# kcheng1021/UC-NeRF

Hardware: AMD Instinct MI355X
Metric: rays/sec (fwd render), 1280x1920 @ 64+128 samples (higher is better)
Workload: dtype f32-class (dense layers: f16 MFMA on hi/lo-split f32 operands, 2^-22 per product, f32 accumulate; grid, resampling, compositing f32)

## Files before the change

ucnerf_amd/_lib.py:

```python
import ctypes
import os

import torch

_HERE = os.path.dirname(os.path.abspath(__file__))
LIB_PATH = os.environ.get("UCN_LIB_PATH") or os.path.join(_HERE, "csrc", "libucnerf_march.so")
ABI_VERSION = 26
LAUNCH_CORESIDENT = 0x100
TABLE_F16 = 0x200
RAYS_INCOHERENT = 0x1000
GFEAT_LEVEL_MAJOR4 = 0x20000
GFEAT_LEVEL_MAJOR = 0x10000
BWD_FIXED_POINT = 0x800
FEATURES_BF16 = 0x400
FEAT_BF16 = 0x100

c_u32, c_u64, c_i32, c_f32, c_vp = ctypes.c_uint32, ctypes.c_uint64, ctypes.c_int, ctypes.c_float, ctypes.c_void_p


class UcnField(ctypes.Structure):
    _fields_ = [
        ("embeddings", c_vp), ("offsets_host", c_vp), ("grid_sizes_host", c_vp),
        ("num_levels", c_u32), ("level_dim", c_u32), ("base_resolution", c_u32),
        ("log2_per_level_scale", c_f32),
        ("w_d0", c_vp), ("b_d0", c_vp), ("w_d1", c_vp), ("b_d1", c_vp),
        ("n_bottleneck", c_u32),
        ("w_c0", c_vp), ("b_c0", c_vp), ("w_c1", c_vp), ("b_c1", c_vp), ("w_rgb", c_vp), ("b_rgb", c_vp),
        ("n_width", c_u32), ("n_dir", c_u32),
        ("density_bias", c_f32), ("rgb_premultiplier", c_f32), ("rgb_bias", c_f32), ("rgb_padding", c_f32),
        ("packed", c_vp),
        ("mlp_mode", c_u32),
    ]


class UcnSky(ctypes.Structure):
    _fields_ = [
        ("w_pts", c_vp * 8), ("b_pts", c_vp * 8),
        ("w_alpha", c_vp), ("b_alpha", c_vp), ("w_feat", c_vp), ("b_feat", c_vp),
        ("w_view", c_vp), ("b_view", c_vp), ("w_rgb", c_vp), ("b_rgb", c_vp),
        ("packed", c_vp),
# ... 155 lines not shown
```

ucnerf_amd/csrc/field_mlp.hip:

```cpp
#include "field_plan.h"
#include "wave_dpp.h"

namespace {

__global__ __launch_bounds__(256) void k_pack_first(const float *__restrict__ W, uint32_t F, float *__restrict__ dst) {
    const uint32_t i = blockIdx.x * 256u + threadIdx.x;
    const uint32_t KQ = F / 2;
    if (i >= 2u * KQ * 64u) return;
    const uint32_t lane = i & 63u, q = (i >> 6) % KQ, ot = (i >> 6) / KQ;
    dst[i] = W[(size_t)(32u * ot + (lane & 31u)) * F + 2u * q + (lane >> 5)];
}

constexpr int kMaxDir = 27;
template <int NW>
__global__ __launch_bounds__(256) void k_dir_bias(const float *__restrict__ viewdirs, const float *__restrict__ wc0,
                                                  const float *__restrict__ wc1, uint32_t nb, uint32_t ndir,
                                                  uint32_t N, float *__restrict__ out) {
    constexpr int RB = 16;
    constexpr int GROUPS = 256 / NW;
    __shared__ float enc[RB][kMaxDir + 1];
    const uint32_t ray0 = blockIdx.x * RB;
    const uint32_t deg = (ndir - 3u) / 6u;
    for (uint32_t i = threadIdx.x; i < RB * ndir; i += 256u) {
        const uint32_t rl = i / ndir, k = i - rl * ndir;
// ... 96 lines not shown
    init_bias<NTB>(x, a.b_d1, nullptr, h);
    chain<NTB, 2>(G1, x, h0, ws);
    if (live && h == 0) a.density[out_index(a, b)] = softplus(x[0][0] + a.density_bias);
    if (a.bott && live) {
#pragma unroll
        for (int t = 0; t < NTB; t++)
#pragma unroll
            for (int r = 0; r < 16; r++) a.bott[(size_t)out_index(a, b) * (NTB * 32) + acc_row(t, r, h)] = x[t][r];
    }
    if (a.rgb == nullptr) {
        ws.drain();
        __syncthreads();
        return;
    }
    const float *db = a.dir_bias + (size_t)ray_index(a, b) * 2 * (NTW * 32);
    f32x16 h2[NTW];
    init_bias<NTW>(h2, a.b_c1, db + NTW * 32, h);
    chain<NTW, NTB>(G2, h2, x, ws);
    hidden_tiles<0, NTB, NTW>(G3, PER_TILE, h2, x, a.b_c0, db, h, ws);
    rgb_head<NTW>(h2, a, b, live, h);
}

}

extern "C" uint64_t ucn_field_packed_floats(const ucn_field_t *f) {
    PackPlan pl;
    if (make_plan(f, &pl)) return 0;
    return pl.total;
}

extern "C" uint64_t ucn_field_dir_floats(const ucn_field_t *f, uint32_t N) {
    PackPlan pl;
    if (make_plan(f, &pl) || pl.prop) return 0;
    return f->mlp_mode == 1 ? (uint64_t)N * 32 : (uint64_t)N * 2 * f->n_width;
}

extern "C" int ucn_field_pack(const ucn_field_t *f, ucn_stream_t stream) {
    PackPlan pl;
    if (int rc = make_plan(f, &pl)) return rc;
    UCN_REQUIRE(f->packed && f->w_d0 && f->w_d1 && f->b_d0 && f->b_d1, "field_pack: density MLP weights / packed buffer missing");
    hipStream_t st = (hipStream_t)stream;
    if (!pl.prop && f->mlp_mode == 1) return ucn_h_pack(f, pl, st);
    hipLaunchKernelGGL(k_pack_first, dim3(ucn_div_up(2ull * pl.KQ * 64, 256)), dim3(256), 0, st, f->w_d0, pl.F, f->packed + pl.p0);
    if (pl.prop) {
        hipLaunchKernelGGL(k_pack_head, dim3(1), dim3(256), 0, st, f->w_d1, 64u, 0u, 64u, 1u, 1u, f->packed + pl.phead);
    } else {
        const uint32_t NB = f->n_bottleneck, NW = f->n_width, ND = f->n_dir;
        uint64_t off = pl.pstream;
        auto chainpack = [&](const float *W, uint32_t ld, uint32_t col0, uint32_t row_tile0, uint32_t nto, uint32_t nti) {
            hipLaunchKernelGGL(k_pack_chain, dim3(ucn_div_up((uint64_t)nto * nti * 1024, 256)), dim3(256), 0, st, W, ld,
                               col0, row_tile0, nto, nti, f->packed + off);
            off += (uint64_t)nto * nti * 1024;
        };
        chainpack(f->w_d1, 64, 0, 0, pl.NTB, 2);
        chainpack(f->w_c1, NW + NB + ND, NW, 0, pl.NTW, pl.NTB);
        for (uint32_t t = 0; t < pl.NTW; t++) {
            chainpack(f->w_c0, NB + ND, 0, t, 1, pl.NTB);
            chainpack(f->w_c1, NW + NB + ND, 32 * t, 0, pl.NTW, 1);
        }
        const uint64_t end = pl.pstream + (uint64_t)pl.n_groups * 256;
        if (off < end)
            hipLaunchKernelGGL(k_fill_zero, dim3(ucn_div_up(end - off, 256)), dim3(256), 0, st, f->packed + off, (uint32_t)(end - off));
        hipLaunchKernelGGL(k_pack_head, dim3(ucn_div_up((uint64_t)NW * 4, 256)), dim3(256), 0, st, f->w_rgb, NW, 0u, NW,
                           3u, 4u, f->packed + pl.phead);
    }
    UCN_LAUNCH_CHECK("field_pack");
    return 0;
}

extern "C" int ucn_field_dir_bias(const ucn_field_t *f, const float *viewdirs, uint32_t N, float *dir_bias_out,
                                  ucn_stream_t stream) {
    PackPlan pl;
    if (int rc = make_plan(f, &pl)) return rc;
    UCN_REQUIRE(!pl.prop, "field_dir_bias: field has no colour MLP (disable_rgb)");
    UCN_REQUIRE(N == 0 || (viewdirs && dir_bias_out), "field_dir_bias: null pointer argument");
    UCN_REQUIRE((f->n_dir - 3) % 6 == 0, "field_dir_bias: n_dir must be 3+6*deg, got %u", f->n_dir);
    if (N == 0) return 0;
    hipStream_t st = (hipStream_t)stream;
    if (f->mlp_mode == 1) return ucn_h_dir_enc(f, viewdirs, N, dir_bias_out, st);
    const dim3 grid(ucn_div_up(N, 16));
    if (f->n_width == 256)
        hipLaunchKernelGGL(k_dir_bias<256>, grid, dim3(256), 0, st, viewdirs, f->w_c0, f->w_c1, f->n_bottleneck, f->n_dir, N, dir_bias_out);
    else
        hipLaunchKernelGGL(k_dir_bias<64>, grid, dim3(256), 0, st, viewdirs, f->w_c0, f->w_c1, f->n_bottleneck, f->n_dir, N, dir_bias_out);
    UCN_LAUNCH_CHECK("field_dir_bias");
    return 0;
}

static thread_local const uint32_t *g_mlp_idx = nullptr, *g_mlp_count = nullptr;

extern "C" int ucn_field_mlp(const ucn_field_t *f, const float *features, uint32_t B, uint32_t samples_per_ray,
                             int rays_fastest, const float *dir_bias, float *density_out, float *rgb_out,
                             float *bottleneck_out, ucn_stream_t stream) {
    PackPlan pl;
    if (int rc = make_plan(f, &pl)) return rc;
    UCN_REQUIRE(B == 0 || (features && density_out && f->packed), "field_mlp: null pointer argument");
    UCN_REQUIRE(samples_per_ray >= 1, "field_mlp: samples_per_ray must be >= 1");
    UCN_REQUIRE(pl.prop ? rgb_out == nullptr : true, "field_mlp: a disable_rgb field has no colour output");
    UCN_REQUIRE(B == 0 || rgb_out == nullptr || dir_bias != nullptr, "field_mlp: colour output needs the per-ray direction terms");
    if (B == 0) return 0;
    MlpArgs a;
    a.feat = features; a.packed = f->packed;
    a.b_d0 = f->b_d0; a.b_d1 = f->b_d1; a.b_c0 = f->b_c0; a.b_c1 = f->b_c1; a.b_rgb = f->b_rgb;
    a.dir_bias = dir_bias; a.density = density_out; a.rgb = rgb_out; a.bott = bottleneck_out;
    UCN_REQUIRE(!(rays_fastest & 1) || B % samples_per_ray == 0, "field_mlp: B must be rays x samples_per_ray");
    a.B = B; a.spr = samples_per_ray; a.C = f->level_dim; a.F = pl.F;
    a.cshift = 0xFFu;
    if ((a.C == 1 || a.C == 2 || a.C == 4 || a.C == 8) && (uint64_t)B * a.C * (pl.F / a.C + 2) < (1ull << 30))
        a.cshift = a.C == 1 ? 0u : a.C == 2 ? 1u : a.C == 4 ? 2u : 3u;
    a.n_rays = B / samples_per_ray; a.rays_fastest = (rays_fastest & 1) ? 1u : 0u;
    a.small_ring = (rays_fastest & UCN_LAUNCH_CORESIDENT) ? 1u : 0u;
    a.idx = g_mlp_idx; a.count = g_mlp_count;
    a.n_chunks = pl.n_groups / kChunkGroups;
    a.p0 = pl.p0; a.pstream = pl.pstream; a.phead = pl.phead;
    a.density_bias = f->density_bias; a.rgb_premult = f->rgb_premultiplier; a.rgb_bias = f->rgb_bias;
    a.rgb_padding = f->rgb_padding;
    const dim3 grid(ucn_div_up(B, 128));
    hipStream_t st = (hipStream_t)stream;
    const size_t lds = 2 * kChunkGroups * 256 * sizeof(float);
    if (pl.prop) hipLaunchKernelGGL(k_prop_mlp, grid, dim3(256), 0, st, a);
    else if (f->mlp_mode == 1) return ucn_h_launch(pl, a, grid, st);
    else if (pl.NTB == 8) hipLaunchKernelGGL((k_field_mlp<8, 8>), grid, dim3(256), lds, st, a);
    else hipLaunchKernelGGL((k_field_mlp<2, 2>), grid, dim3(256), lds, st, a);
    UCN_LAUNCH_CHECK("field_mlp");
    return 0;
}

extern "C" int ucn_field_rgb_compacted(const ucn_field_t *f, const float *features, uint32_t B, uint32_t samples_per_ray,
                                       int rays_fastest, const float *dir_bias, const uint32_t *idx, const uint32_t *count,
                                       float *rgb_out, ucn_stream_t stream) {
    UCN_REQUIRE(f && f->mlp_mode == 1 && f->n_bottleneck != 1, "field_rgb_compacted: needs a colour field in mlp_mode 1");
    UCN_REQUIRE(B == 0 || (idx && count && rgb_out), "field_rgb_compacted: null pointer argument");
    g_mlp_idx = idx; g_mlp_count = count;
    const int rc = ucn_field_mlp(f, features, B, samples_per_ray, rays_fastest, dir_bias, rgb_out, rgb_out, nullptr, stream);
    g_mlp_idx = g_mlp_count = nullptr;
    return rc;
}
```

ucnerf_amd/csrc/field_mlp_h.hip:

```cpp
#include "field_plan.h"
#include "wave_dpp.h"
#include "mlp_ring.h"

namespace {

constexpr int kKS = (int)kFirstSteps;
constexpr int kDirExp = 10;
enum { E_IN = 0, E_H0 = 1, E_H1 = 2, E_H2 = 3, E_COUNT = 4 };

__global__ __launch_bounds__(256) void k_dir_enc(const float *__restrict__ viewdirs, uint32_t ndir, uint32_t N,
                                                 float *__restrict__ out) {
    const uint32_t i = blockIdx.x * 256u + threadIdx.x;
    if (i >= N * 32u) return;
    const uint32_t ray = i >> 5, k = i & 31u;
    const uint32_t deg = (ndir - 3u) / 6u;
    float v;
    if (k < 3u) {
        v = viewdirs[ray * 3 + k];
    } else if (k < ndir) {
        const uint32_t kk = (k - 3u) % (3u * deg), a = kk % 3u, si = kk / 3u;
        const float sc = viewdirs[ray * 3 + a] * (float)(1u << si);
        v = (k - 3u) < 3u * deg ? sinf(sc) : sinf(sc + 1.5707963705062866f);
    } else {
        v = k == ndir ? 1.0f : 0.0f;
    }
    out[i] = ldexpf(v, kDirExp);
}

__global__ __launch_bounds__(256) void k_compose(const float *__restrict__ Wout, uint32_t ldo, uint32_t col0,
                                                 const float *__restrict__ bias_out, const float *__restrict__ Wd1,
                                                 const float *__restrict__ bd1, uint32_t NB, uint32_t ND, uint32_t NW,
                                                 float *__restrict__ M) {
    const uint32_t i = blockIdx.x * 256u + threadIdx.x;
    if (i >= NW * kCompCols) return;
    const uint32_t j = i / kCompCols, c = i - j * kCompCols;
    const float *wr = Wout + (size_t)j * ldo + col0;
    float v = 0.0f;
    if (c < 64u) {
        double acc = 0.0;
        for (uint32_t k = 0; k < NB; k++) acc += (double)wr[k] * (double)Wd1[(size_t)k * 64 + c];
        v = (float)acc;
    } else if (c - 64u < ND) {
        v = wr[NB + c - 64u];
    } else if (c == 64u + ND) {
        double acc = (double)bias_out[j];
        for (uint32_t k = 0; k < NB; k++) acc += (double)wr[k] * (double)bd1[k];
        v = (float)acc;
    }
    M[i] = v;
}

__global__ __launch_bounds__(256) void k_absmax(const float *__restrict__ x, uint64_t n, uint32_t *__restrict__ out_bits) {
    float m = 0.0f;
    for (uint64_t i = (uint64_t)blockIdx.x * 256u + threadIdx.x; i < n; i += (uint64_t)gridDim.x * 256u) {
        const float v = fabsf(x[i]);
        m = v > m ? v : m;
    }
#pragma unroll
    for (int o = 32; o > 0; o >>= 1) m = fmaxf(m, __shfl_xor(m, o, 64));
// ... 158 lines not shown
#else
#define UCN_STAMP(i) do { } while (0)
#endif
template <int NTW, bool RGB, int CHUNK, int STAGE>
__global__ __launch_bounds__(256) void k_field_mlp_h(MlpArgs a) {
#ifdef UCN_EXP_TIMING
    const unsigned long long t_begin = __builtin_readcyclecounter();
#endif
    extern __shared__ __attribute__((aligned(16))) float s_lds[];
    const int lane = threadIdx.x & 63;
    const int wave = __builtin_amdgcn_readfirstlane(threadIdx.x >> 6);
    const int j = lane & 31, h = lane >> 5;
    const uint32_t b0 = (blockIdx.x * 4u + wave) * 32u;
    bool live = b0 + j < a.B;
    uint32_t b = live ? b0 + j : a.B - 1;
    if (a.idx) {
        const uint32_t cnt = *a.count;
        if (blockIdx.x * 128u >= cnt) return;
        live = b0 + j < cnt;
        b = a.idx[live ? b0 + j : cnt - 1];
    }
    const uint32_t oi = out_index(a, b);

    constexpr int NP = NTW / 2;
    constexpr int GA = 4 * kKS;
    constexpr int GB = GA + NP * 24;
    constexpr int PB = 24 + NTW * 8;
    constexpr int NG = RGB ? GB + NP * PB : GA;

    float fv[kKS][8];
    load_features<kKS>(a, b, h, fv);
    f32x16 ev;
    if constexpr (RGB) {
        const float4 *ep = reinterpret_cast<const float4 *>(a.dir_bias + (size_t)ray_index(a, b) * 32 + 4 * h);
#pragma unroll
        for (int r4 = 0; r4 < 4; r4++) {
            const float4 v = ep[2 * r4];
            ev[4 * r4 + 0] = v.x; ev[4 * r4 + 1] = v.y; ev[4 * r4 + 2] = v.z; ev[4 * r4 + 3] = v.w;
        }
    }
    const float *side = s_lds;
    Ring<NG, CHUNK, 4, kRingSlots, kLead, STAGE> ring(a.packed + a.pstream + kSideGroups * 256, s_lds + kSideGroups * 256, lane, wave);
    {
        const uint32_t lbase = (uint32_t)(size_t)(__attribute__((address_space(3))) float *)s_lds;
#pragma unroll
        for (int i = 0; i < kSideGroups / 4; i++)
            dma_group(a.packed + a.pstream + (size_t)(i * 4 + wave) * 256, lbase + (uint32_t)(i * 4 + wave) * 1024u, (uint32_t)lane * 16u);
    }
    rstatic_for<kLead>([&](auto c) { ring.template issue_chunk<c.value>(); });
    UCN_STAMP(0);
    if constexpr (STAGE > 0) ring.drain();
    ring.template boundary<0>();
    UCN_STAMP(1);
    if constexpr (RGB) {
#pragma unroll
        for (int r = 0; r < 16; r++) asm volatile("" : "+v"(ev[r]));
    }
    const float in_scale = side[129];

    f32x16 acc0[2];
#pragma unroll
    for (int t = 0; t < 2; t++) {
        const float4 *pb = reinterpret_cast<const float4 *>(side + t * 32 + h * 16);
#pragma unroll
        for (int r4 = 0; r4 < 4; r4++) {
            const float4 v = pb[r4];
            acc0[t][4 * r4 + 0] = v.x; acc0[t][4 * r4 + 1] = v.y; acc0[t][4 * r4 + 2] = v.z; acc0[t][4 * r4 + 3] = v.w;
// ... 68 lines not shown
                    dstep<G, NG>(acc[qp][0], acc[qp][1], in[i / 2].hi[i % 2], in[i / 2].lo[i % 2], pipe, ring);
            });
            UCN_STAMP(5 + 2 * p);
            rstatic_for<2 * NTW>([&](auto ic) {
                constexpr int i = ic.value, G = GB + p * PB + 24 + i * 4;
                if constexpr (p > 0 && i < 2)
                    dstep<G, NG, 3, 4>(acc[qp][0], acc[qp][1], h1s[i / 2].hi[i % 2], h1s[i / 2].lo[i % 2], pipe, ring,
                                       [&] { head_eighth<2 * (p - 1), 6 + i>(acc[qq], side, h, s0, s1, s2); });
                else
                    dstep<G, NG>(acc[qp][0], acc[qp][1], h1s[i / 2].hi[i % 2], h1s[i / 2].lo[i % 2], pipe, ring);
            });
            UCN_STOP_AT(3 + p, acc[qp]);
        });
        UCN_STAMP(13);
        rstatic_for<8>([&](auto e) { head_eighth<2 * (NP - 1), e.value>(acc[(2 * NP - 1) % 2], side, h, s0, s1, s2); });
        UCN_STAMP(14);
        s0 = xor32_sum(s0);
        s1 = xor32_sum(s1);
        s2 = xor32_sum(s2);
        if (live && h == 0) {
            const float pad = a.rgb_padding;
            const float v[3] = {s0 + a.b_rgb[0], s1 + a.b_rgb[1], s2 + a.b_rgb[2]};
            const size_t o = (size_t)oi * 3;
#pragma unroll
            for (int c = 0; c < 3; c++) {
                const float sg = 1.0f / (1.0f + expf(-(a.rgb_premult * v[c] + a.rgb_bias)));
                a.rgb[o + c] = sg * (1.0f + 2.0f * pad) - pad;
            }
        }
    }
}


template <int NTW, int NWAVES, int CHUNK, int SLOTS, int LEAD, int DEPTH>
__global__ __launch_bounds__(NWAVES * 64, 2) void k_field_mlp_h8(MlpArgs a) {
#ifdef UCN_EXP_TIMING
    const unsigned long long t_begin = __builtin_readcyclecounter();
#define UCN_STAMP8(i) do { if (blockIdx.x == UCN_EXP_TIMING && (threadIdx.x & 255) == 0) a.bott[(threadIdx.x >> 8) * 32 + (i)] = (float)(__builtin_readcyclecounter() - t_begin); } while (0)
#else
#define UCN_STAMP8(i) do { } while (0)
#endif
    extern __shared__ __attribute__((aligned(16))) float s_lds[];
    const int lane = threadIdx.x & 63;
    const int wave = __builtin_amdgcn_readfirstlane(threadIdx.x >> 6);
    const int j = lane & 31, h = lane >> 5;
    const uint32_t b0 = (blockIdx.x * NWAVES + wave) * 32u;
    bool live = b0 + j < a.B;
    uint32_t b = live ? b0 + j : a.B - 1;
    if (a.idx) {
        const uint32_t cnt = *a.count;
        if (blockIdx.x * (NWAVES * 32u) >= cnt) return;
        live = b0 + j < cnt;
        b = a.idx[live ? b0 + j : cnt - 1];
    }
    const uint32_t oi = out_index(a, b);
    constexpr int NP = NTW / 2;
    constexpr int GA = 4 * kKS;
    constexpr int GB = GA + NP * 24;
    constexpr int PB = 24 + NTW * 8;
    constexpr int NG = GB + NP * PB;

    float fv[kKS][8];
    load_features<kKS>(a, b, h, fv);
    f32x16 ev;
    {
        const float4 *ep = reinterpret_cast<const float4 *>(a.dir_bias + (size_t)ray_index(a, b) * 32 + 4 * h);
#pragma unroll
        for (int r4 = 0; r4 < 4; r4++) {
            const float4 v = ep[2 * r4];
            ev[4 * r4 + 0] = v.x; ev[4 * r4 + 1] = v.y; ev[4 * r4 + 2] = v.z; ev[4 * r4 + 3] = v.w;
        }
    }
    const float *side = s_lds;
    Ring<NG, CHUNK, NWAVES, SLOTS, LEAD> ring(a.packed + a.pstream + kSideGroups * 256, s_lds + kSideGroups * 256, lane, wave);
    {
        const uint32_t lbase = (uint32_t)(size_t)(__attribute__((address_space(3))) float *)s_lds;
#pragma unroll
        for (int i = 0; i < kSideGroups / NWAVES; i++)
            dma_group(a.packed + a.pstream + (size_t)(i * NWAVES + wave) * 256, lbase + (uint32_t)(i * NWAVES + wave) * 1024u, (uint32_t)lane * 16u);
    }
    UCN_STAMP8(0);
    rstatic_for<LEAD>([&](auto c) { ring.template issue_chunk<c.value>(); });
    UCN_STAMP8(1);
    ring.template boundary<0>();
    UCN_STAMP8(2);
#pragma unroll
    for (int r = 0; r < 16; r++) asm volatile("" : "+v"(ev[r]));
    const float in_scale = side[129];

    f32x16 acc[2];
#pragma unroll
    for (int t = 0; t < 2; t++) {
        const float4 *pb = reinterpret_cast<const float4 *>(side + t * 32 + h * 16);
#pragma unroll
        for (int r4 = 0; r4 < 4; r4++) {
            const float4 v = pb[r4];
            acc[t][4 * r4 + 0] = v.x; acc[t][4 * r4 + 1] = v.y; acc[t][4 * r4 + 2] = v.z; acc[t][4 * r4 + 3] = v.w;
        }
    }
    OpPipeD<DEPTH> pipe;
    pipe_prime_d<NG>(pipe, ring);
    {
        h8 fhi[kKS], flo[kKS];
#pragma unroll
        for (int s = 0; s < kKS; s++) {
#pragma unroll
            for (int e = 0; e < 8; e++) fv[s][e] *= in_scale;
            rsplit8(fv[s], fhi[s], flo[s]);
        }
        rstatic_for<kKS>([&](auto s) { dstep_d<4 * s.value, NG>(acc[0], acc[1], fhi[s.value], flo[s.value], pipe, ring); });
    }
    {
        const float *pd = side + 64;
        float part = 0.0f;
#pragma unroll
        for (int it = 0; it < 2; it++)
#pragma unroll
            for (int r = 0; r < 16; r++) part = fmaf(relu_bits(acc[it][r]), pd[(it * 16 + r) * 2 + h], part);
        const float raw = xor32_sum(part) + pd[64];
        if (live && h == 0 && a.idx == nullptr) a.density[oi] = softplus(raw + a.density_bias);
    }
    UCN_STAMP8(3);
    HPair in[3];
#pragma unroll
    for (int s = 0; s < 2; s++) {
        split_half<true>(acc[0], s, in[0]);
        split_half<true>(acc[1], s, in[1]);
        split_half<false>(ev, s, in[2]);
    }
    UCN_STAMP8(4);
    HPair h1s[NTW];
    rstatic_for<NP>([&](auto pc) {
        constexpr int p = pc.value;
#pragma unroll
        for (int r = 0; r < 16; r++) acc[0][r] = acc[1][r] = 0.0f;
        rstatic_for<6>([&](auto ic) {
            constexpr int i = ic.value, G = GA + (p * 6 + i) * 4;
            dstep_d<G, NG>(acc[0], acc[1], in[i / 2].hi[i % 2], in[i / 2].lo[i % 2], pipe, ring);
        });
#pragma unroll
        for (int s = 0; s < 2; s++) {
            split_half<true>(acc[0], s, h1s[2 * p]);
            split_half<true>(acc[1], s, h1s[2 * p + 1]);
        }
    });
    UCN_STAMP8(5);
    float s0 = 0.0f, s1 = 0.0f, s2 = 0.0f;
    rstatic_for<NP>([&](auto pc) {
        constexpr int p = pc.value;
#pragma unroll
        for (int r = 0; r < 16; r++) acc[0][r] = acc[1][r] = 0.0f;
        rstatic_for<6>([&](auto ic) {
            constexpr int i = ic.value, G = GB + p * PB + i * 4;
            dstep_d<G, NG>(acc[0], acc[1], in[i / 2].hi[i % 2], in[i / 2].lo[i % 2], pipe, ring);
        });
        rstatic_for<2 * NTW>([&](auto ic) {
            constexpr int i = ic.value, G = GB + p * PB + 24 + i * 4;
            dstep_d<G, NG>(acc[0], acc[1], h1s[i / 2].hi[i % 2], h1s[i / 2].lo[i % 2], pipe, ring);
        });
        UCN_STAMP8(6 + 2 * p);
        rstatic_for<8>([&](auto e) { head_eighth<2 * p, e.value>(acc, side, h, s0, s1, s2); });
        UCN_STAMP8(7 + 2 * p);
    });
    s0 = xor32_sum(s0);
    s1 = xor32_sum(s1);
    s2 = xor32_sum(s2);
    if (live && h == 0) {
        const float pad = a.rgb_padding;
        const float v[3] = {s0 + a.b_rgb[0], s1 + a.b_rgb[1], s2 + a.b_rgb[2]};
        const size_t o = (size_t)oi * 3;
#pragma unroll
        for (int c = 0; c < 3; c++) {
            const float sg = 1.0f / (1.0f + expf(-(a.rgb_premult * v[c] + a.rgb_bias)));
            a.rgb[o + c] = sg * (1.0f + 2.0f * pad) - pad;
        }
    }
}

}

int ucn_h_pack(const ucn_field_t *f, const PackPlan &pl, hipStream_t st) {
    const uint32_t NB = f->n_bottleneck, NW = f->n_width, ND = f->n_dir;
    float *side = f->packed + pl.pstream;
    float *stream = side + kSideGroups * 256;
    float *MA = f->packed + pl.pcomp, *MB = MA + (size_t)NW * kCompCols;
    float *scratch = MB + (size_t)NW * kCompCols;
    int *exps = reinterpret_cast<int *>(scratch + 1);
    const uint64_t n_floats = (uint64_t)pl.n_groups * 256;
    hipLaunchKernelGGL(k_fill_zero, dim3(ucn_div_up(n_floats, 256)), dim3(256), 0, st, side, (uint32_t)n_floats);
    hipLaunchKernelGGL(k_fill_zero, dim3(1), dim3(256), 0, st, scratch, 16u);
    const dim3 cg(ucn_div_up((uint64_t)NW * kCompCols, 256));
    hipLaunchKernelGGL(k_compose, cg, dim3(256), 0, st, f->w_c0, NB + ND, 0u, f->b_c0, f->w_d1, f->b_d1, NB, ND, NW, MA);
    hipLaunchKernelGGL(k_compose, cg, dim3(256), 0, st, f->w_c1, NW + NB + ND, NW, f->b_c1, f->w_d1, f->b_d1, NB, ND, NW, MB);
    const uint64_t n_emb = (uint64_t)f->offsets_host[f->num_levels] * f->level_dim;
    hipLaunchKernelGGL(k_absmax, dim3(1024), dim3(256), 0, st, f->embeddings, n_emb, reinterpret_cast<uint32_t *>(scratch));
    hipLaunchKernelGGL(k_field_scales, dim3(1), dim3(256), 0, st, f->w_d0, f->b_d0, pl.F, MA, MB, f->w_c1, NW + NB + ND, NW, ND,
                       reinterpret_cast<const uint32_t *>(scratch), exps, side, scratch + 8);
    hipLaunchKernelGGL(k_pack_side, dim3(ucn_div_up(256u + NW * 4u, 256)), dim3(256), 0, st, f->b_d0, f->w_d1, f->b_d1, f->w_rgb, NW,
                       exps, side);
    uint64_t g = 0;
    auto pairs = [&](const float *W, uint32_t ld, uint32_t row_tile0, uint32_t nto, uint32_t nti, int e_out, int e_lo,
                     uint32_t split_col) {
        hipLaunchKernelGGL(k_pack_pairs, dim3(ucn_div_up((uint64_t)nto * nti * 2048, 256)), dim3(256), 0, st, W, ld, 0u,
                           row_tile0, nto, nti, exps, e_out, e_lo, split_col, kDirExp, reinterpret_cast<_Float16 *>(stream + g * 256));
        g += (uint64_t)nto * nti * 4;
    };
    hipLaunchKernelGGL(k_pack_first_s, dim3(ucn_div_up(2ull * kFirstSteps * 1024, 256)), dim3(256), 0, st, f->w_d0, pl.F,
                       kFirstSteps, exps, reinterpret_cast<_Float16 *>(stream));
    g += 2 * kFirstSteps * 2;
    pairs(MA, kCompCols, 0, pl.NTW, 3, E_H1, E_H0, 64u);
    for (uint32_t otp = 0; otp < pl.NTW / 2; otp++) {
        pairs(MB, kCompCols, 2 * otp, 2, 3, E_H2, E_H0, 64u);
        pairs(f->w_c1, NW + NB + ND, 2 * otp, 2, pl.NTW, E_H2, E_H1, 0xFFFFFFFFu);
    }
    UCN_REQUIRE(g == stream_groups_h(pl.NTW), "field_pack: internal stream length mismatch (%llu)", (unsigned long long)g);
    UCN_LAUNCH_CHECK("field_pack (split-f16)");
    return 0;
}

int ucn_h_dir_enc(const ucn_field_t *f, const float *viewdirs, uint32_t N, float *out, hipStream_t st) {
    hipLaunchKernelGGL(k_dir_enc, dim3(ucn_div_up((uint64_t)N * 32, 256)), dim3(256), 0, st, viewdirs, f->n_dir, N, out);
    UCN_LAUNCH_CHECK("field_dir_bias (split-f16)");
    return 0;
}

int ucn_h_launch(const PackPlan &pl, const MlpArgs &a, dim3 grid, hipStream_t st) {
#ifndef UCN_EXP_TIMING
    UCN_REQUIRE(a.bott == nullptr, "field_mlp: mlp_mode 1 composes the bottleneck away; request bottleneck_out with mlp_mode 0");
#endif
#define UCN_MLP_H(NTW_, RGB_)                                                                                              \
    do {                                                                                                                   \
        if (a.small_ring)                                                                                                  \
            hipLaunchKernelGGL((k_field_mlp_h<NTW_, RGB_, kRingChunkSmall, 0>), grid, dim3(256), ring_lds_bytes(kRingChunkSmall), st, a); \
        else                                                                                                               \
            hipLaunchKernelGGL((k_field_mlp_h<NTW_, RGB_, kRingChunk, UCN_MLP4_STAGE>), grid, dim3(256), ring_lds_bytes(kRingChunk), st, a); \
    } while (0)
#ifndef UCN_MLP8_DEPTH
#define UCN_MLP8_DEPTH 2
#endif
#ifndef UCN_MLP4_STAGE
#define UCN_MLP4_STAGE 0
#endif
#ifndef UCN_MLP8_CHUNK
#define UCN_MLP8_CHUNK 32
#define UCN_MLP8_SLOTS 4
#define UCN_MLP8_LEAD 2
#endif
#ifndef UCN_MLP2_CHUNK
#define UCN_MLP2_CHUNK 16
#define UCN_MLP2_SLOTS 4
#define UCN_MLP2_LEAD 2
#endif
    static const int waves = getenv("UCN_MLP_WAVES") ? atoi(getenv("UCN_MLP_WAVES")) : 4;
    if (a.rgb != nullptr && pl.NTW == 8 && !a.small_ring && waves == 8) {
        const dim3 grid8(ucn_div_up(a.B, 256));
        hipLaunchKernelGGL((k_field_mlp_h8<8, 8, UCN_MLP8_CHUNK, UCN_MLP8_SLOTS, UCN_MLP8_LEAD, UCN_MLP8_DEPTH>), grid8, dim3(512),
                           (kSideGroups + UCN_MLP8_SLOTS * UCN_MLP8_CHUNK) * 1024, st, a);
        UCN_LAUNCH_CHECK("field_mlp (split-f16, 8 waves)");
        return 0;
    }
    if (a.rgb != nullptr && pl.NTW == 8 && (waves == 4 || a.small_ring)) {
        hipLaunchKernelGGL((k_field_mlp_h8<8, 4, UCN_MLP2_CHUNK, UCN_MLP2_SLOTS, UCN_MLP2_LEAD, UCN_MLP8_DEPTH>), grid, dim3(256),
                           (kSideGroups + UCN_MLP2_SLOTS * UCN_MLP2_CHUNK) * 1024, st, a);
        UCN_LAUNCH_CHECK("field_mlp (split-f16, 2 workgroups per CU)");
        return 0;
    }
    if (a.rgb == nullptr) {
        if (pl.NTW == 8) UCN_MLP_H(8, false);
        else UCN_MLP_H(2, false);
    } else {
        if (pl.NTW == 8) UCN_MLP_H(8, true);
        else UCN_MLP_H(2, true);
    }
#undef UCN_MLP_H
    UCN_LAUNCH_CHECK("field_mlp (split-f16)");
    return 0;
}
```

ucnerf_amd/csrc/field_plan.h:

```cpp
#pragma once
#include "mfma_chain.h"
#include "wave_dpp.h"
#include "mlp_ring.h"

struct PackPlan {
    uint64_t p0, pstream, phead, pcomp, total;
    uint32_t F, KQ, NTB, NTW, n_groups;
    bool prop;
};

static inline uint32_t stream_groups_f32(uint32_t NTB, uint32_t NTW) {
    return NTB * 2 * 4 + NTW * NTB * 4 + NTW * (NTB * 4 + NTW * 4);
}
constexpr uint32_t kFirstSteps = 4;
constexpr uint32_t kCompCols = 96;
static inline uint32_t stream_groups_h(uint32_t NTW) {
    return 4 * (kFirstSteps + 3 * NTW + NTW * (3 + NTW));
}

static inline int make_plan(const ucn_field_t *f, PackPlan *pl) {
    UCN_REQUIRE(f, "field: null descriptor");
    UCN_REQUIRE(f->mlp_mode <= 1, "field: mlp_mode must be 0 (fp32 MFMA) or 1 (split-f16 MFMA)");
    pl->F = f->num_levels * f->level_dim;
    UCN_REQUIRE(pl->F % 2 == 0 && pl->F >= 2, "field: num_levels*level_dim must be even, got %u", pl->F);
    pl->KQ = pl->F / 2;
    pl->prop = f->n_bottleneck == 1;
    pl->p0 = 0;
    uint64_t o = 2ull * pl->KQ * 64;
    const uint64_t o_h = 2ull * ((pl->F + 15) / 16) * 2 * 256;
    if (o_h > o) o = o_h;
    o = (o + 255) & ~255ull;
    if (pl->prop) {
        pl->NTB = pl->NTW = 0;
        pl->n_groups = 0;
        pl->pstream = o;
        pl->phead = o; o += 64;
        pl->pcomp = o;
    } else {
        UCN_REQUIRE((f->n_bottleneck == 256 && f->n_width == 256) || (f->n_bottleneck == 64 && f->n_width == 64),
                    "field: supported (bottleneck_width, net_width_viewdirs) are (256,256) and (64,64), got (%u,%u)",
                    f->n_bottleneck, f->n_width);
        UCN_REQUIRE(f->w_c0 && f->w_c1 && f->w_rgb && f->b_c0 && f->b_c1 && f->b_rgb, "field: colour MLP weights missing");
        UCN_REQUIRE(f->n_dir >= 3 && f->n_dir <= 27, "field: n_dir must be in [3,27] (one 32-wide tile incl. the bias slot)");
        UCN_REQUIRE(f->mlp_mode == 0 || pl->F <= 16 * kFirstSteps,
                    "field: mlp_mode 1 supports num_levels*level_dim <= %u, got %u", 16 * kFirstSteps, pl->F);
        pl->NTB = f->n_bottleneck / 32;
        pl->NTW = f->n_width / 32;
        const uint32_t g0 = (stream_groups_f32(pl->NTB, pl->NTW) + kChunkGroups - 1) / kChunkGroups * kChunkGroups;
        const uint32_t g1 = kSideGroups + (stream_groups_h(pl->NTW) + kRingPad - 1) / kRingPad * kRingPad + kRingPad;
        pl->n_groups = f->mlp_mode == 1 ? g1 : g0;
        pl->pstream = o; o += (uint64_t)(g0 > g1 ? g0 : g1) * 256;
        pl->phead = o; o += (uint64_t)pl->NTW * 128;
        pl->pcomp = o; o += 2ull * f->n_width * kCompCols + 16;
    }
    pl->total = o;
    return 0;
}

struct MlpArgs {
    const float *feat;
    const float *packed;
    const float *b_d0, *b_d1, *b_c0, *b_c1, *b_rgb;
    const float *dir_bias;
    float *density, *rgb, *bott;
    uint32_t B, spr, C, F, n_chunks;
    uint32_t cshift;
    uint32_t n_rays, rays_fastest;
    uint32_t small_ring;
    const uint32_t *idx, *count;
    uint64_t p0, pstream, phead;
    float density_bias, rgb_premult, rgb_bias, rgb_padding;
};

template <int KS>
__device__ __forceinline__ void load_features(const MlpArgs &a, uint32_t b, int h, float (&fv)[KS][8]) {
    if (a.cshift != 0xFFu) {
        const uint32_t BC = a.B * a.C, cm = a.C - 1u;
        const uint32_t mine = b * a.C + (uint32_t)h * ((8u >> a.cshift) * BC);
        const bool whole = (a.F & 15u) == 0u;
#pragma unroll
        for (int s = 0; s < KS; s++)
#pragma unroll
            for (int e = 0; e < 8; e++) {
                const uint32_t kk = 16u * s + e;
                const float *row = a.feat + ((size_t)(kk >> a.cshift) * BC + (kk & cm));
                const bool ok = whole ? kk < a.F : kk + 8u * h < a.F;
                fv[s][e] = ok ? row[mine] : 0.0f;
            }
        return;
    }
#pragma unroll
    for (int s = 0; s < KS; s++)
#pragma unroll
        for (int e = 0; e < 8; e++) {
            const uint32_t k = 16u * s + 8u * h + e, l = k / a.C, c = k - l * a.C;
            fv[s][e] = k < a.F ? a.feat[((size_t)l * a.B + b) * a.C + c] : 0.0f;
        }
}

__device__ __forceinline__ uint32_t ray_index(const MlpArgs &a, uint32_t b) {
    return a.rays_fastest ? b % a.n_rays : b / a.spr;
// ... 5 lines not shown
    return x > 20.0f ? x : log1pf(expf(x));
}

template <int NTW>
__device__ __forceinline__ void rgb_head(const f32x16 (&h2)[NTW], const MlpArgs &a, uint32_t b, bool live, int h) {
    const float4 *pr = reinterpret_cast<const float4 *>(a.packed + a.phead);
    float s0 = 0.0f, s1 = 0.0f, s2 = 0.0f;
#pragma unroll
    for (int t = 0; t < NTW; t++)
#pragma unroll
        for (int r = 0; r < 16; r++) {
            const float4 w = pr[(t * 16 + r) * 2 + h];
            const float v = fmaxf(h2[t][r], 0.0f);
            s0 = fmaf(v, w.x, s0);
            s1 = fmaf(v, w.y, s1);
            s2 = fmaf(v, w.z, s2);
        }
    s0 = xor32_sum(s0);
    s1 = xor32_sum(s1);
    s2 = xor32_sum(s2);
    if (live && h == 0) {
        const float pad = a.rgb_padding;
        float v[3] = {s0 + a.b_rgb[0], s1 + a.b_rgb[1], s2 + a.b_rgb[2]};
        const size_t o = (size_t)out_index(a, b) * 3;
#pragma unroll
        for (int c = 0; c < 3; c++) {
            const float sg = 1.0f / (1.0f + expf(-(a.rgb_premult * v[c] + a.rgb_bias)));
            a.rgb[o + c] = sg * (1.0f + 2.0f * pad) - pad;
        }
    }
}

int ucn_h_pack(const ucn_field_t *f, const PackPlan &pl, hipStream_t st);
int ucn_h_dir_enc(const ucn_field_t *f, const float *viewdirs, uint32_t N, float *out, hipStream_t st);
int ucn_h_launch(const PackPlan &pl, const MlpArgs &a, dim3 grid, hipStream_t st);
```

ucnerf_amd/csrc/grid_op.hip:

```cpp
#include <stdarg.h>

#include "ucn_common.h"

thread_local char g_ucn_err[512] = {0};

int ucn_fail(const char *fmt, ...) {
    va_list ap;
    va_start(ap, fmt);
    vsnprintf(g_ucn_err, sizeof(g_ucn_err), fmt, ap);
    va_end(ap);
    return 1;
}

extern "C" const char *ucn_last_error(void) { return g_ucn_err; }
extern "C" uint32_t ucn_abi_version(void) { return 26; }

int ucn_build_levels(UcnLevels *out, const int32_t *offsets, const int32_t *grid_sizes, uint32_t L, uint32_t C,
                     uint32_t D, float S, uint32_t H, uint32_t gridtype, int align_corners) {
    UCN_REQUIRE(L >= 1 && L <= UCN_MAX_LEVELS, "GridEncoding: num_levels must be in [1,%d], got %u", UCN_MAX_LEVELS, L);
    UCN_REQUIRE(D >= 2 && D <= 5, "GridEncoding: D must be 2, 3, 4 or 5.");
    memset(out, 0, sizeof(*out));
    out->L = L;
    out->C = C;
    for (uint32_t l = 0; l < L; l++) {
        UcnLevel &lv = out->lv[l];
        UCN_REQUIRE(offsets[l + 1] > offsets[l], "GridEncoding: offsets must be increasing");
        lv.first_row = (uint32_t)offsets[l];
        lv.rows = (uint32_t)(offsets[l + 1] - offsets[l]);
        lv.scale = exp2f((float)l * S) * (float)H - 1.0f;
        lv.resolution = (uint32_t)ceilf(lv.scale) + 1u;
        lv.mask = (lv.rows & (lv.rows - 1)) == 0 ? lv.rows - 1 : 0;
        const uint32_t side = align_corners ? lv.resolution : lv.resolution + 1u;
        uint32_t stride = 1;
        for (uint32_t d = 0; d < D && stride <= lv.rows; d++) {
            lv.stride[d] = stride;
            stride *= side;
        }
        lv.hashed = (gridtype == 0u && stride > lv.rows) ? 1u : 0u;
        if (grid_sizes) {
            const int32_t g = grid_sizes[l];
            lv.gs2 = (float)(int32_t)((uint32_t)g * (uint32_t)g);
            lv.inv_gs = 1.0f / sqrtf(lv.gs2);
        }
    }
    return 0;
}

namespace {
// ... 441 lines not shown
```

Measured before the change: 5.449 million.

## Precompute per-ray direction terms and seed MLP accumulators with ray-tiled launch

Adds a kernel that computes each ray's direction-encoding contribution to both colour hidden layers once per ray and stores it alongside the encoding. The fused MLP kernel then starts its accumulators from these precomputed terms, so it no longer runs the direction-input MFMA steps for every sample. It also adds a ray-tile launch mode in which each wave handles 32 samples of one ray and DMAs that ray's terms into LDS. The cost is a larger per-ray buffer (32+512 floats), a second packed weight stream with one fewer input, and more kernel variants to maintain.

```diff
diff --git a/ucnerf_amd/_lib.py b/ucnerf_amd/_lib.py
--- a/ucnerf_amd/_lib.py
+++ b/ucnerf_amd/_lib.py
@@ -5,7 +5,7 @@
 
 _HERE = os.path.dirname(os.path.abspath(__file__))
 LIB_PATH = os.environ.get("UCN_LIB_PATH") or os.path.join(_HERE, "csrc", "libucnerf_march.so")
-ABI_VERSION = 26
+ABI_VERSION = 27
 LAUNCH_CORESIDENT = 0x100
 TABLE_F16 = 0x200
 RAYS_INCOHERENT = 0x1000
diff --git a/ucnerf_amd/csrc/field_mlp.hip b/ucnerf_amd/csrc/field_mlp.hip
--- a/ucnerf_amd/csrc/field_mlp.hip
+++ b/ucnerf_amd/csrc/field_mlp.hip
@@ -152,7 +152,7 @@
 extern "C" uint64_t ucn_field_dir_floats(const ucn_field_t *f, uint32_t N) {
     PackPlan pl;
     if (make_plan(f, &pl) || pl.prop) return 0;
-    return f->mlp_mode == 1 ? (uint64_t)N * 32 : (uint64_t)N * 2 * f->n_width;
+    return f->mlp_mode == 1 ? (uint64_t)N * dir_stride_h(f->n_width) : (uint64_t)N * 2 * f->n_width;
 }
 
 extern "C" int ucn_field_pack(const ucn_field_t *f, ucn_stream_t stream) {
@@ -197,7 +197,7 @@
     UCN_REQUIRE((f->n_dir - 3) % 6 == 0, "field_dir_bias: n_dir must be 3+6*deg, got %u", f->n_dir);
     if (N == 0) return 0;
     hipStream_t st = (hipStream_t)stream;
-    if (f->mlp_mode == 1) return ucn_h_dir_enc(f, viewdirs, N, dir_bias_out, st);
+    if (f->mlp_mode == 1) return ucn_h_dir_enc(f, pl, viewdirs, N, dir_bias_out, st);
     const dim3 grid(ucn_div_up(N, 16));
     if (f->n_width == 256)
         hipLaunchKernelGGL(k_dir_bias<256>, grid, dim3(256), 0, st, viewdirs, f->w_c0, f->w_c1, f->n_bottleneck, f->n_dir, N, dir_bias_out);
@@ -231,6 +231,7 @@
     a.n_rays = B / samples_per_ray; a.rays_fastest = (rays_fastest & 1) ? 1u : 0u;
     a.small_ring = (rays_fastest & UCN_LAUNCH_CORESIDENT) ? 1u : 0u;
     a.idx = g_mlp_idx; a.count = g_mlp_count;
+    a.dstride = dir_stride_h(f->n_width); a.prt = 0;
     a.n_chunks = pl.n_groups / kChunkGroups;
     a.p0 = pl.p0; a.pstream = pl.pstream; a.phead = pl.phead;
     a.density_bias = f->density_bias; a.rgb_premult = f->rgb_premultiplier; a.rgb_bias = f->rgb_bias;
diff --git a/ucnerf_amd/csrc/field_mlp_h.hip b/ucnerf_amd/csrc/field_mlp_h.hip
--- a/ucnerf_amd/csrc/field_mlp_h.hip
+++ b/ucnerf_amd/csrc/field_mlp_h.hip
@@ -25,6 +25,51 @@
         v = k == ndir ? 1.0f : 0.0f;
     }
     out[i] = ldexpf(v, kDirExp);
+}
+
+__global__ __launch_bounds__(256) void k_dir_terms(const float *__restrict__ viewdirs, const float *__restrict__ MA,
+                                                   const float *__restrict__ MB, const int *__restrict__ exps, uint32_t ndir,
+                                                   uint32_t N, float *__restrict__ out) {
+    constexpr uint32_t RB = 32, STRIDE = 32 + 512;
+    __shared__ float enc[RB][32];
+    const uint32_t ray0 = blockIdx.x * RB;
+    const uint32_t deg = (ndir - 3u) / 6u;
+    for (uint32_t i = threadIdx.x; i < RB * 32u; i += 256u) {
+        const uint32_t rl = i >> 5, k = i & 31u;
+        const uint32_t ray = ray0 + rl < N ? ray0 + rl : N - 1;
+        float v;
+        if (k < 3u) {
+            v = viewdirs[ray * 3 + k];
+        } else if (k < ndir) {
+            const uint32_t kk = (k - 3u) % (3u * deg), a = kk % 3u, si = kk / 3u;
+            const float sc = viewdirs[ray * 3 + a] * (float)(1u << si);
+            v = (k - 3u) < 3u * deg ? sinf(sc) : sinf(sc + 1.5707963705062866f);
+        } else {
+            v = k == ndir ? 1.0f : 0.0f;
+        }
+        enc[rl][k] = v;
+        if (ray0 + rl < N) out[(size_t)(ray0 + rl) * STRIDE + k] = ldexpf(v, kDirExp);
+    }
+    __syncthreads();
+    const uint32_t t = threadIdx.x >> 5, h = (threadIdx.x >> 4) & 1u, r = threadIdx.x & 15u;
+    const uint32_t n = acc_row(t, r, h);
+    float wa[28], wb[28];
+#pragma unroll
+    for (uint32_t k = 0; k < 28u; k++) {
+        wa[k] = k <= ndir ? ldexpf(MA[n * kCompCols + 64u + k], exps[E_H1]) : 0.0f;
+        wb[k] = k <= ndir ? ldexpf(MB[n * kCompCols + 64u + k], exps[E_H2]) : 0.0f;
+    }
+    for (uint32_t rl = 0; rl < RB && ray0 + rl < N; rl++) {
+        float sa = 0.0f, sb = 0.0f;
+#pragma unroll
+        for (uint32_t k = 0; k < 28u; k++) {
+            sa = fmaf(wa[k], enc[rl][k], sa);
+            sb = fmaf(wb[k], enc[rl][k], sb);
+        }
+        float *o = out + (size_t)(ray0 + rl) * STRIDE + 32u + threadIdx.x;
+        o[0] = sa;
+        o[256] = sb;
+    }
 }
 
 __global__ __launch_bounds__(256) void k_compose(const float *__restrict__ Wout, uint32_t ldo, uint32_t col0,
@@ -249,7 +294,7 @@
     load_features<kKS>(a, b, h, fv);
     f32x16 ev;
     if constexpr (RGB) {
-        const float4 *ep = reinterpret_cast<const float4 *>(a.dir_bias + (size_t)ray_index(a, b) * 32 + 4 * h);
+        const float4 *ep = reinterpret_cast<const float4 *>(a.dir_bias + (size_t)ray_index(a, b) * a.dstride + 4 * h);
 #pragma unroll
         for (int r4 = 0; r4 < 4; r4++) {
             const float4 v = ep[2 * r4];
@@ -384,8 +429,11 @@
 }
 
 
-template <int NTW, int NWAVES, int CHUNK, int SLOTS, int LEAD, int DEPTH>
+constexpr int kSideUsed = 5;
+constexpr int kRtLdsGroups = kSideUsed + 8;
+template <int NTW, int NWAVES, int CHUNK, int SLOTS, int LEAD, int DEPTH, int MODE>
 __global__ __launch_bounds__(NWAVES * 64, 2) void k_field_mlp_h8(MlpArgs a) {
+    constexpr bool RT = MODE == 1, SEEDED = MODE != 0;
 #ifdef UCN_EXP_TIMING
     const unsigned long long t_begin = __builtin_readcyclecounter();
 #define UCN_STAMP8(i) do { if (blockIdx.x == UCN_EXP_TIMING && (threadIdx.x & 255) == 0) a.bott[(threadIdx.x >> 8) * 32 + (i)] = (float)(__builtin_readcyclecounter() - t_begin); } while (0)
@@ -396,27 +444,50 @@
     const int lane = threadIdx.x & 63;
     const int wave = __builtin_amdgcn_readfirstlane(threadIdx.x >> 6);
     const int j = lane & 31, h = lane >> 5;
-    const uint32_t b0 = (blockIdx.x * NWAVES + wave) * 32u;
-    bool live = b0 + j < a.B;
-    uint32_t b = live ? b0 + j : a.B - 1;
-    if (a.idx) {
-        const uint32_t cnt = *a.count;
-        if (blockIdx.x * (NWAVES * 32u) >= cnt) return;
-        live = b0 + j < cnt;
-        b = a.idx[live ? b0 + j : cnt - 1];
-    }
-    const uint32_t oi = out_index(a, b);
+    bool live;
+    uint32_t b, oi, ray = 0;
+    if constexpr (RT) {
+        static_assert(NWAVES == 4, "ray tiles: four neighbouring rays per workgroup");
+        const uint32_t tiles = a.spr >> 5;
+        uint32_t s0;
+        if (a.rays_fastest) {
+            const uint32_t groups = (a.n_rays + 3u) >> 2, st = blockIdx.x / groups;
+            ray = (blockIdx.x - st * groups) * 4u + wave;
+            s0 = st * 32u;
+        } else {
+            const uint32_t t = blockIdx.x * 4u + wave;
+            ray = t / tiles;
+            s0 = (t - ray * tiles) * 32u;
+        }
+        live = ray < a.n_rays;
+        ray = live ? ray : a.n_rays - 1;
+        b = a.rays_fastest ? (s0 + j) * a.n_rays + ray : ray * a.spr + s0 + j;
+        oi = ray * a.spr + s0 + j;
+    } else {
+        const uint32_t b0 = (blockIdx.x * NWAVES + wave) * 32u;
+        live = b0 + j < a.B;
+        b = live ? b0 + j : a.B - 1;
+        if (a.idx) {
+            const uint32_t cnt = *a.count;
+            if (blockIdx.x * (NWAVES * 32u) >= cnt) return;
+            live = b0 + j < cnt;
+            b = a.idx[live ? b0 + j : cnt - 1];
+        }
+        oi = out_index(a, b);
+    }
     constexpr int NP = NTW / 2;
+    constexpr int NI = SEEDED ? 2 : 3;
     constexpr int GA = 4 * kKS;
-    constexpr int GB = GA + NP * 24;
-    constexpr int PB = 24 + NTW * 8;
+    constexpr int GB = GA + NP * NI * 8;
+    constexpr int PB = NI * 8 + NTW * 8;
     constexpr int NG = GB + NP * PB;
+    constexpr int SIDE = RT ? kSideUsed : kSideGroups, RING0 = RT ? kRtLdsGroups : kSideGroups;
 
     float fv[kKS][8];
     load_features<kKS>(a, b, h, fv);
     f32x16 ev;
-    {
-        const float4 *ep = reinterpret_cast<const float4 *>(a.dir_bias + (size_t)ray_index(a, b) * 32 + 4 * h);
+    if constexpr (!SEEDED) {
+        const float4 *ep = reinterpret_cast<const float4 *>(a.dir_bias + (size_t)ray_index(a, b) * a.dstride + 4 * h);
 #pragma unroll
         for (int r4 = 0; r4 < 4; r4++) {
             const float4 v = ep[2 * r4];
@@ -424,20 +495,44 @@
         }
     }
     const float *side = s_lds;
-    Ring<NG, CHUNK, NWAVES, SLOTS, LEAD> ring(a.packed + a.pstream + kSideGroups * 256, s_lds + kSideGroups * 256, lane, wave);
+    Ring<NG, CHUNK, NWAVES, SLOTS, LEAD> ring(a.packed + (SEEDED ? a.prt : a.pstream + kSideGroups * 256), s_lds + RING0 * 256, lane, wave);
     {
         const uint32_t lbase = (uint32_t)(size_t)(__attribute__((address_space(3))) float *)s_lds;
 #pragma unroll
-        for (int i = 0; i < kSideGroups / NWAVES; i++)
-            dma_group(a.packed + a.pstream + (size_t)(i * NWAVES + wave) * 256, lbase + (uint32_t)(i * NWAVES + wave) * 1024u, (uint32_t)lane * 16u);
-    }
+        for (int i = 0; i < (SIDE + NWAVES - 1) / NWAVES; i++)
+            if (SIDE % NWAVES == 0 || i * NWAVES + wave < SIDE)
+                dma_group(a.packed + a.pstream + (size_t)(i * NWAVES + wave) * 256, lbase + (uint32_t)(i * NWAVES + wave) * 1024u, (uint32_t)lane * 16u);
+        if constexpr (RT) {
+            const float *g = a.dir_bias + (size_t)ray * a.dstride + 32;
+#pragma unroll
+            for (int q = 0; q < 2; q++)
+                dma_group(g + q * 256, lbase + (uint32_t)((kSideUsed + 2 * wave + q) * 1024), (uint32_t)lane * 16u);
+        }
+    }
+    const float *seeds = RT ? s_lds + (kSideUsed + 2 * wave) * 256 + h * 16
+                            : a.dir_bias + (SEEDED ? (size_t)ray_index(a, b) * a.dstride + 32 + h * 16 : 0);
+    auto seed = [&](f32x16 &acc_, int L, int T) {
+        if constexpr (SEEDED) {
+            const float4 *ps = reinterpret_cast<const float4 *>(seeds + (L * NTW + T) * 32);
+#pragma unroll
+            for (int r4 = 0; r4 < 4; r4++) {
+                const float4 v = ps[r4];
+                acc_[4 * r4 + 0] = v.x; acc_[4 * r4 + 1] = v.y; acc_[4 * r4 + 2] = v.z; acc_[4 * r4 + 3] = v.w;
+            }
+        } else {
+#pragma unroll
+            for (int r = 0; r < 16; r++) acc_[r] = 0.0f;
+        }
+    };
     UCN_STAMP8(0);
     rstatic_for<LEAD>([&](auto c) { ring.template issue_chunk<c.value>(); });
     UCN_STAMP8(1);
     ring.template boundary<0>();
     UCN_STAMP8(2);
-#pragma unroll
-    for (int r = 0; r < 16; r++) asm volatile("" : "+v"(ev[r]));
+    if constexpr (!SEEDED) {
+#pragma unroll
+        for (int r = 0; r < 16; r++) asm volatile("" : "+v"(ev[r]));
+    }
     const float in_scale = side[129];
 
     f32x16 acc[2];
@@ -473,21 +568,21 @@
         if (live && h == 0 && a.idx == nullptr) a.density[oi] = softplus(raw + a.density_bias);
     }
     UCN_STAMP8(3);
-    HPair in[3];
+    HPair in[NI];
 #pragma unroll
     for (int s = 0; s < 2; s++) {
         split_half<true>(acc[0], s, in[0]);
         split_half<true>(acc[1], s, in[1]);
-        split_half<false>(ev, s, in[2]);
+        if constexpr (!SEEDED) split_half<false>(ev, s, in[2]);
     }
     UCN_STAMP8(4);
     HPair h1s[NTW];
     rstatic_for<NP>([&](auto pc) {
         constexpr int p = pc.value;
-#pragma unroll
-        for (int r = 0; r < 16; r++) acc[0][r] = acc[1][r] = 0.0f;
-        rstatic_for<6>([&](auto ic) {
-            constexpr int i = ic.value, G = GA + (p * 6 + i) * 4;
+        seed(acc[0], 0, 2 * p);
+        seed(acc[1], 0, 2 * p + 1);
+        rstatic_for<2 * NI>([&](auto ic) {
+            constexpr int i = ic.value, G = GA + (p * 2 * NI + i) * 4;
             dstep_d<G, NG>(acc[0], acc[1], in[i / 2].hi[i % 2], in[i / 2].lo[i % 2], pipe, ring);
         });
 #pragma unroll
@@ -500,14 +595,14 @@
     float s0 = 0.0f, s1 = 0.0f, s2 = 0.0f;
     rstatic_for<NP>([&](auto pc) {
         constexpr int p = pc.value;
-#pragma unroll
-        for (int r = 0; r < 16; r++) acc[0][r] = acc[1][r] = 0.0f;
-        rstatic_for<6>([&](auto ic) {
+        seed(acc[0], 1, 2 * p);
+        seed(acc[1], 1, 2 * p + 1);
+        rstatic_for<2 * NI>([&](auto ic) {
             constexpr int i = ic.value, G = GB + p * PB + i * 4;
             dstep_d<G, NG>(acc[0], acc[1], in[i / 2].hi[i % 2], in[i / 2].lo[i % 2], pipe, ring);
         });
         rstatic_for<2 * NTW>([&](auto ic) {
-            constexpr int i = ic.value, G = GB + p * PB + 24 + i * 4;
+            constexpr int i = ic.value, G = GB + p * PB + NI * 8 + i * 4;
             dstep_d<G, NG>(acc[0], acc[1], h1s[i / 2].hi[i % 2], h1s[i / 2].lo[i % 2], pipe, ring);
         });
         UCN_STAMP8(6 + 2 * p);
@@ -557,21 +652,32 @@
                            row_tile0, nto, nti, exps, e_out, e_lo, split_col, kDirExp, reinterpret_cast<_Float16 *>(stream + g * 256));
         g += (uint64_t)nto * nti * 4;
     };
-    hipLaunchKernelGGL(k_pack_first_s, dim3(ucn_div_up(2ull * kFirstSteps * 1024, 256)), dim3(256), 0, st, f->w_d0, pl.F,
-                       kFirstSteps, exps, reinterpret_cast<_Float16 *>(stream));
-    g += 2 * kFirstSteps * 2;
-    pairs(MA, kCompCols, 0, pl.NTW, 3, E_H1, E_H0, 64u);
-    for (uint32_t otp = 0; otp < pl.NTW / 2; otp++) {
-        pairs(MB, kCompCols, 2 * otp, 2, 3, E_H2, E_H0, 64u);
-        pairs(f->w_c1, NW + NB + ND, 2 * otp, 2, pl.NTW, E_H2, E_H1, 0xFFFFFFFFu);
-    }
-    UCN_REQUIRE(g == stream_groups_h(pl.NTW), "field_pack: internal stream length mismatch (%llu)", (unsigned long long)g);
+    for (uint32_t n_in = 3; n_in >= (pl.rt_group ? 2u : 3u); n_in--) {
+        const uint64_t g_first = n_in == 3 ? 0 : pl.rt_group - kSideGroups;
+        g = g_first;
+        hipLaunchKernelGGL(k_pack_first_s, dim3(ucn_div_up(2ull * kFirstSteps * 1024, 256)), dim3(256), 0, st, f->w_d0, pl.F,
+                           kFirstSteps, exps, reinterpret_cast<_Float16 *>(stream + g * 256));
+        g += 2 * kFirstSteps * 2;
+        pairs(MA, kCompCols, 0, pl.NTW, n_in, E_H1, E_H0, 64u);
+        for (uint32_t otp = 0; otp < pl.NTW / 2; otp++) {
+            pairs(MB, kCompCols, 2 * otp, 2, n_in, E_H2, E_H0, 64u);
+            pairs(f->w_c1, NW + NB + ND, 2 * otp, 2, pl.NTW, E_H2, E_H1, 0xFFFFFFFFu);
+        }
+        UCN_REQUIRE(g - g_first == stream_groups_h(pl.NTW, n_in), "field_pack: internal stream length mismatch (%llu)", (unsigned long long)g);
+    }
     UCN_LAUNCH_CHECK("field_pack (split-f16)");
     return 0;
 }
 
-int ucn_h_dir_enc(const ucn_field_t *f, const float *viewdirs, uint32_t N, float *out, hipStream_t st) {
-    hipLaunchKernelGGL(k_dir_enc, dim3(ucn_div_up((uint64_t)N * 32, 256)), dim3(256), 0, st, viewdirs, f->n_dir, N, out);
+int ucn_h_dir_enc(const ucn_field_t *f, const PackPlan &pl, const float *viewdirs, uint32_t N, float *out, hipStream_t st) {
+    if (dir_stride_h(f->n_width) != 32) {
+        UCN_REQUIRE(f->packed, "field_dir_bias: mlp_mode 1 reads the composed matrices of ucn_field_pack (packed is null)");
+        const float *MA = f->packed + pl.pcomp, *MB = MA + (size_t)f->n_width * kCompCols;
+        const int *exps = reinterpret_cast<const int *>(MB + (size_t)f->n_width * kCompCols + 1);
+        hipLaunchKernelGGL(k_dir_terms, dim3(ucn_div_up(N, 32)), dim3(256), 0, st, viewdirs, MA, MB, exps, f->n_dir, N, out);
+    } else {
+        hipLaunchKernelGGL(k_dir_enc, dim3(ucn_div_up((uint64_t)N * 32, 256)), dim3(256), 0, st, viewdirs, f->n_dir, N, out);
+    }
     UCN_LAUNCH_CHECK("field_dir_bias (split-f16)");
     return 0;
 }
@@ -604,15 +710,34 @@
 #define UCN_MLP2_LEAD 2
 #endif
     static const int waves = getenv("UCN_MLP_WAVES") ? atoi(getenv("UCN_MLP_WAVES")) : 4;
+    const char *rt_env = getenv("UCN_MLP_RAY_TILE");
+    const bool ray_tiles = !(rt_env && atoi(rt_env) == 0);
+    const bool tiles_ok = a.rgb != nullptr && pl.NTW == 8 && waves == 4 && ray_tiles && a.spr % 32u == 0u && a.B == a.n_rays * a.spr;
+    MlpArgs rt = a;
+    rt.prt = a.pstream + (uint64_t)pl.rt_group * 256;
+    if (tiles_ok && (a.small_ring || a.idx != nullptr)) {
+        hipLaunchKernelGGL((k_field_mlp_h8<8, 4, UCN_MLP2_CHUNK, UCN_MLP2_SLOTS, UCN_MLP2_LEAD, UCN_MLP8_DEPTH, 2>), grid, dim3(256),
+                           (kSideGroups + UCN_MLP2_SLOTS * UCN_MLP2_CHUNK) * 1024, st, rt);
+        UCN_LAUNCH_CHECK("field_mlp (split-f16, per-lane direction terms)");
+        return 0;
+    }
+    if (tiles_ok) {
+        const uint32_t tiles = a.spr / 32u;
+        const dim3 grid_rt(a.rays_fastest ? ucn_div_up(a.n_rays, 4) * tiles : ucn_div_up((uint64_t)a.n_rays * tiles, 4));
+        hipLaunchKernelGGL((k_field_mlp_h8<8, 4, UCN_MLP2_CHUNK, UCN_MLP2_SLOTS, UCN_MLP2_LEAD, UCN_MLP8_DEPTH, 1>), grid_rt, dim3(256),
+                           (kRtLdsGroups + UCN_MLP2_SLOTS * UCN_MLP2_CHUNK) * 1024, st, rt);
+        UCN_LAUNCH_CHECK("field_mlp (split-f16, ray tiles)");
+        return 0;
+    }
     if (a.rgb != nullptr && pl.NTW == 8 && !a.small_ring && waves == 8) {
         const dim3 grid8(ucn_div_up(a.B, 256));
-        hipLaunchKernelGGL((k_field_mlp_h8<8, 8, UCN_MLP8_CHUNK, UCN_MLP8_SLOTS, UCN_MLP8_LEAD, UCN_MLP8_DEPTH>), grid8, dim3(512),
+        hipLaunchKernelGGL((k_field_mlp_h8<8, 8, UCN_MLP8_CHUNK, UCN_MLP8_SLOTS, UCN_MLP8_LEAD, UCN_MLP8_DEPTH, 0>), grid8, dim3(512),
                            (kSideGroups + UCN_MLP8_SLOTS * UCN_MLP8_CHUNK) * 1024, st, a);
         UCN_LAUNCH_CHECK("field_mlp (split-f16, 8 waves)");
         return 0;
     }
     if (a.rgb != nullptr && pl.NTW == 8 && (waves == 4 || a.small_ring)) {
-        hipLaunchKernelGGL((k_field_mlp_h8<8, 4, UCN_MLP2_CHUNK, UCN_MLP2_SLOTS, UCN_MLP2_LEAD, UCN_MLP8_DEPTH>), grid, dim3(256),
+        hipLaunchKernelGGL((k_field_mlp_h8<8, 4, UCN_MLP2_CHUNK, UCN_MLP2_SLOTS, UCN_MLP2_LEAD, UCN_MLP8_DEPTH, 0>), grid, dim3(256),
                            (kSideGroups + UCN_MLP2_SLOTS * UCN_MLP2_CHUNK) * 1024, st, a);
         UCN_LAUNCH_CHECK("field_mlp (split-f16, 2 workgroups per CU)");
         return 0;
diff --git a/ucnerf_amd/csrc/field_plan.h b/ucnerf_amd/csrc/field_plan.h
--- a/ucnerf_amd/csrc/field_plan.h
+++ b/ucnerf_amd/csrc/field_plan.h
@@ -6,6 +6,7 @@
 struct PackPlan {
     uint64_t p0, pstream, phead, pcomp, total;
     uint32_t F, KQ, NTB, NTW, n_groups;
+    uint32_t rt_group;
     bool prop;
 };
 
@@ -14,9 +15,13 @@
 }
 constexpr uint32_t kFirstSteps = 4;
 constexpr uint32_t kCompCols = 96;
-static inline uint32_t stream_groups_h(uint32_t NTW) {
-    return 4 * (kFirstSteps + 3 * NTW + NTW * (3 + NTW));
+static inline uint32_t stream_groups_h(uint32_t NTW, uint32_t n_in = 3) {
+    return 4 * (kFirstSteps + n_in * NTW + NTW * (n_in + NTW));
 }
+static inline uint32_t ring_padded(uint32_t groups) {
+    return (groups + kRingPad - 1) / kRingPad * kRingPad + kRingPad;
+}
+static inline uint32_t dir_stride_h(uint32_t n_width) { return n_width == 256 ? 32 + 2 * n_width : 32; }
 
 static inline int make_plan(const ucn_field_t *f, PackPlan *pl) {
     UCN_REQUIRE(f, "field: null descriptor");
@@ -32,7 +37,7 @@
     o = (o + 255) & ~255ull;
     if (pl->prop) {
         pl->NTB = pl->NTW = 0;
-        pl->n_groups = 0;
+        pl->n_groups = pl->rt_group = 0;
         pl->pstream = o;
         pl->phead = o; o += 64;
         pl->pcomp = o;
@@ -47,7 +52,8 @@
         pl->NTB = f->n_bottleneck / 32;
         pl->NTW = f->n_width / 32;
         const uint32_t g0 = (stream_groups_f32(pl->NTB, pl->NTW) + kChunkGroups - 1) / kChunkGroups * kChunkGroups;
-        const uint32_t g1 = kSideGroups + (stream_groups_h(pl->NTW) + kRingPad - 1) / kRingPad * kRingPad + kRingPad;
+        pl->rt_group = pl->NTW == 8 ? kSideGroups + ring_padded(stream_groups_h(pl->NTW)) : 0;
+        const uint32_t g1 = kSideGroups + ring_padded(stream_groups_h(pl->NTW)) + (pl->NTW == 8 ? ring_padded(stream_groups_h(pl->NTW, 2)) : 0);
         pl->n_groups = f->mlp_mode == 1 ? g1 : g0;
         pl->pstream = o; o += (uint64_t)(g0 > g1 ? g0 : g1) * 256;
         pl->phead = o; o += (uint64_t)pl->NTW * 128;
@@ -67,6 +73,8 @@
     uint32_t cshift;
     uint32_t n_rays, rays_fastest;
     uint32_t small_ring;
+    uint32_t dstride;
+    uint64_t prt;
     const uint32_t *idx, *count;
     uint64_t p0, pstream, phead;
     float density_bias, rgb_premult, rgb_bias, rgb_padding;
@@ -138,5 +146,5 @@
 }
 
 int ucn_h_pack(const ucn_field_t *f, const PackPlan &pl, hipStream_t st);
-int ucn_h_dir_enc(const ucn_field_t *f, const float *viewdirs, uint32_t N, float *out, hipStream_t st);
+int ucn_h_dir_enc(const ucn_field_t *f, const PackPlan &pl, const float *viewdirs, uint32_t N, float *out, hipStream_t st);
 int ucn_h_launch(const PackPlan &pl, const MlpArgs &a, dim3 grid, hipStream_t st);
diff --git a/ucnerf_amd/csrc/grid_op.hip b/ucnerf_amd/csrc/grid_op.hip
--- a/ucnerf_amd/csrc/grid_op.hip
+++ b/ucnerf_amd/csrc/grid_op.hip
@@ -13,7 +13,7 @@
 }
 
 extern "C" const char *ucn_last_error(void) { return g_ucn_err; }
-extern "C" uint32_t ucn_abi_version(void) { return 26; }
+extern "C" uint32_t ucn_abi_version(void) { return 27; }
 
 int ucn_build_levels(UcnLevels *out, const int32_t *offsets, const int32_t *grid_sizes, uint32_t L, uint32_t C,
                      uint32_t D, float S, uint32_t H, uint32_t gridtype, int align_corners) {
```

New measurement: 5.513 million, median of 6. 1.01x the previous value.
